# RubenMovsesyan/DiPs

Hardware: AMD Instinct MI355X
Metric: frames/s + achieved HBM GB/s (% of roofline), 4K RGB8, 1/2/4/8 GPUs (higher is better)
Workload: dtype u8

## Files before the change

### dips_amd/csrc/dips_abi.hip

```cpp
#include <hip/hip_runtime.h>

#include <cmath>
#include <cstring>
#include <mutex>
#include <new>
#include <string>

#include "dips_handle.h"

namespace {

std::mutex g_err_mu;
std::string g_create_err;

void set_create_err(const std::string& m) {
    std::lock_guard<std::mutex> lk(g_err_mu);
    g_create_err = m;
}

dips_status validate_params(const dips_params* p, std::string* why) {
    if (p->spatial_window_size < 1 || p->spatial_window_size > 11) {
        *why = "spatial_window_size must be in [1, 11] (dips_shader.wgsl:27 MAX_WIN_SIZE_SQUARE = 11*11)";
        return DIPS_ERR_INVALID;
    }
    if (p->chroma_filter > 3u) {
        *why = "chroma_filter must be 0..3 (dips/src/lib.rs:43-61)";
        return DIPS_ERR_INVALID;
    }
    if (p->mode > 1u) {
        *why = "mode must be DIPS_MODE_OVERALL or DIPS_MODE_PER_FRAME";
        return DIPS_ERR_INVALID;
    }
    if (p->format != DIPS_FMT_GRAY8 && p->format != DIPS_FMT_RGB8 && p->format != DIPS_FMT_RGBA8) {
        *why = "format must be DIPS_FMT_GRAY8, DIPS_FMT_RGB8 or DIPS_FMT_RGBA8";
        return DIPS_ERR_INVALID;
    }
    if (!(p->tau >= 0.0f) || std::isinf(p->tau)) {
        *why = "tau must be finite and >= 0";
        return DIPS_ERR_INVALID;
    }
    if (!std::isfinite(p->sensitivity)) {
        *why = "sensitivity must be finite";
        return DIPS_ERR_INVALID;
    }
    return DIPS_OK;
}

}

namespace dips_abi {

void note_error(dips_handle* h, const char* msg) noexcept {
    if (!h) return;
    try {
        h->err = msg;
    } catch (...) {
    }
}

void note_error(CreateTag, const char* msg) noexcept {
    try {
        set_create_err(msg);
    } catch (...) {
    }
}

}

namespace dips_internal {

dips_status fail(dips_handle* h, dips_status st, const std::string& msg) {
    if (h) h->err = msg;
    return st;
}

dips_status hip_fail(dips_handle* h, hipError_t e, const char* what) {
    std::string m = std::string(what) + ": " + hipGetErrorString(e);
    return fail(h, e == hipErrorOutOfMemory ? DIPS_ERR_NOMEM : DIPS_ERR_HIP, m);
}

dips_status bind(dips_handle* h) {
    if (!h) return DIPS_ERR_INVALID;
    hipError_t e = hipSetDevice(h->device);
    if (e != hipSuccess) return hip_fail(h, e, "hipSetDevice");
    return DIPS_OK;
}

hipEvent_t take_event(dips_handle* h) {
    if (!h->ev_free.empty()) {
        hipEvent_t e = h->ev_free.back();
        h->ev_free.pop_back();
        return e;
    }
    hipEvent_t e = nullptr;
    if (hipEventCreate(&e) != hipSuccess) return nullptr;
    return e;
}

int occupancy_blocks(dips_handle* h, const void* kernel) {
    auto it = h->occupancy.find(kernel);
    if (it != h->occupancy.end()) return it->second;
    int nb = 0;
    if (hipOccupancyMaxActiveBlocksPerMultiprocessor(&nb, kernel, 256, 0) != hipSuccess || nb < 1) nb = 1;
    h->occupancy[kernel] = nb;
    return nb;
}

}

using dips_abi::guard;
using namespace dips_internal;

namespace dips_abi {
int current_device() noexcept {
    int d = -1;
    return hipGetDevice(&d) == hipSuccess ? d : -1;
}
void set_device(int dev) noexcept { (void)hipSetDevice(dev); }
}

extern "C" {

int dips_abi_version(void) {
    return guard(nullptr, [&]() -> int { return DIPS_ABI_VERSION; });
}

dips_status dips_params_default(dips_params* p) {
    return guard(nullptr, [&]() -> dips_status {
        if (!p) return DIPS_ERR_INVALID;
        std::memset(p, 0, sizeof(*p));
        p->colorize = 0;
        p->spatial_window_size = 1;
        p->sensitivity = 5.0f;
        p->filter_type = DIPS_FILTER_UNFILTERED;
        p->chroma_filter = DIPS_CHROMA_NONE;
        p->mode = DIPS_MODE_OVERALL;
        p->format = DIPS_FMT_RGB8;
        p->tau = 0.0f;
        p->flags = 0;
        return DIPS_OK;
    });
}

dips_status dips_create(const dips_params* params, int device, dips_handle** out) {
    return guard(dips_abi::CreateTag{}, [&]() -> dips_status {
        if (!out) return DIPS_ERR_INVALID;
        *out = nullptr;
        dips_params p;
        if (params) p = *params;
        else dips_params_default(&p);
        std::string why;
        if (validate_params(&p, &why) != DIPS_OK) {
            set_create_err(why);
            return DIPS_ERR_INVALID;
        }
        int count = 0;
        hipError_t e = hipGetDeviceCount(&count);
        if (e != hipSuccess || count <= 0 || device < 0 || device >= count) {
            set_create_err(std::string("no HIP device ") + std::to_string(device) + " (" +
                           (e == hipSuccess ? std::to_string(count) + " visible" : hipGetErrorString(e)) + ")");
            return DIPS_ERR_NODEVICE;
        }
        dips_handle* h = new (std::nothrow) dips_handle();
        if (!h) return DIPS_ERR_NOMEM;
        h->p = p;
        h->device = device;
        e = hipSetDevice(device);
        if (e == hipSuccess) e = hipDeviceGetAttribute(&h->cu_count, hipDeviceAttributeMultiprocessorCount, device);
        if (e == hipSuccess) e = hipStreamCreateWithFlags(&h->own_stream, hipStreamDefault);
        if (e == hipSuccess) e = hipStreamCreateWithFlags(&h->copy_stream, hipStreamNonBlocking);
        for (int i = 0; i < 3 && e == hipSuccess; ++i) {
            e = hipEventCreateWithFlags(&h->copy_done[i], hipEventDisableTiming);
            if (e == hipSuccess) e = hipEventCreateWithFlags(&h->kernel_done[i], hipEventDisableTiming);
        }
        if (e != hipSuccess) {
            set_create_err(std::string("HIP initialisation failed: ") + hipGetErrorString(e));
            dips_destroy(h);
            return DIPS_ERR_HIP;
        }
        h->stream = h->own_stream;
        *out = h;
        return DIPS_OK;
    });
}

void dips_destroy(dips_handle* h) {
    guard(h, [&]() -> void {
        if (!h) return;
        (void)hipSetDevice(h->device);
        if (h->stream) (void)hipStreamSynchronize(h->stream);
        if (h->copy_stream) (void)hipStreamSynchronize(h->copy_stream);
        if (h->comm_stream) (void)hipStreamSynchronize(h->comm_stream);
        for (auto& pr : h->ev_pending) {
            (void)hipEventDestroy(pr.first);
            (void)hipEventDestroy(pr.second);
        }
        for (auto e : h->ev_free) (void)hipEventDestroy(e);
        for (int i = 0; i < 3; ++i) {
            if (h->copy_done[i]) (void)hipEventDestroy(h->copy_done[i]);
            if (h->kernel_done[i]) (void)hipEventDestroy(h->kernel_done[i]);
            h->ring[i].release();
        }
        h->ring_ref.release();
        h->pinned[0].release();
        h->pinned[1].release();
        h->partials.release();
        h->stage_frames.release();
        h->stage_ref.release();
        h->stage_series.release();
        h->stage_map.release();
        for (auto& s : h->slots) s.release();
        for (auto& s : h->slots_alt) s.release();
        h->pipe.release();
        h->pieces.release();
        h->up_pieces.release();
        h->probe_out.release();
        h->times_parts.release();
        h->cc_scratch.release();
        h->io_out.release();
        h->raw.release();
        h->filtered.release();
        h->cb_lut.release();
        h->gray_lut.release();
        h->start.release();
        h->out.release();
        h->io.release();
        h->shard_ref.release();
        h->shard_halo.release();
        h->shard_send.release();
        h->shard_recv.release();
        h->shard_send_frame.release();
        if (h->comm_stream) (void)hipStreamDestroy(h->comm_stream);
        if (h->shard_ev_in) (void)hipEventDestroy(h->shard_ev_in);
        if (h->shard_ev_halo) (void)hipEventDestroy(h->shard_ev_halo);
        if (h->switch_ev) (void)hipEventDestroy(h->switch_ev);
        if (h->join_ev) (void)hipEventDestroy(h->join_ev);
        if (h->own_stream) (void)hipStreamDestroy(h->own_stream);
        if (h->copy_stream) (void)hipStreamDestroy(h->copy_stream);
        delete h;
    });
}

const char* dips_last_error(const dips_handle* h) {
    return guard(h, [&]() -> const char* {
        if (h) return h->err.c_str();
        thread_local std::string copy;
        std::lock_guard<std::mutex> lk(g_err_mu);
        copy = g_create_err;
        return copy.c_str();
    });
}

dips_status dips_set_stream(dips_handle* h, void* stream) {
    return guard(h, [&]() -> dips_status {
        if (!h) return DIPS_ERR_INVALID;
        hipStream_t next = stream ? static_cast<hipStream_t>(stream) : h->own_stream;
        if (next == h->stream) return DIPS_OK;
        dips_status st = bind(h);
        if (st != DIPS_OK) return st;
        st = flush_pending(h);
        if (st != DIPS_OK) return st;
        if (!h->switch_ev) DIPS_HIP(h, hipEventCreateWithFlags(&h->switch_ev, hipEventDisableTiming));
        DIPS_HIP(h, hipEventRecord(h->switch_ev, h->stream));
        DIPS_HIP(h, hipStreamWaitEvent(next, h->switch_ev, 0));
        h->stream = next;
        return DIPS_OK;
    });
}

dips_status dips_synchronize(dips_handle* h) {
    return guard(h, [&]() -> dips_status {
        dips_status st = bind(h);
        if (st != DIPS_OK) return st;
        st = flush_pending(h);
        if (st != DIPS_OK) return st;
        DIPS_HIP(h, hipStreamSynchronize(h->stream));
        return DIPS_OK;
    });
}

dips_status dips_kernel_time(dips_handle* h, double* total_ms, uint64_t* launches) {
    return guard(h, [&]() -> dips_status {
        dips_status st = bind(h);
        if (st != DIPS_OK) return st;
        for (auto& pr : h->ev_pending) {
            DIPS_HIP(h, hipEventSynchronize(pr.second));
            float ms = 0.0f;
            DIPS_HIP(h, hipEventElapsedTime(&ms, pr.first, pr.second));
            h->t_ms += ms;
            h->t_launches += 1;
            if (h->t_each.size() >= dips_handle::kTimeKeep)
                h->t_each.erase(h->t_each.begin(), h->t_each.begin() + dips_handle::kTimeKeep / 2);
            h->t_each.push_back(ms);
            h->ev_free.push_back(pr.first);
            h->ev_free.push_back(pr.second);
        }
        h->ev_pending.clear();
        if (total_ms) *total_ms = h->t_ms;
        if (launches) *launches = h->t_launches;
        return DIPS_OK;
    });
}

dips_status dips_kernel_time_reset(dips_handle* h) {
    return guard(h, [&]() -> dips_status {
        dips_status st = dips_kernel_time(h, nullptr, nullptr);
        if (st != DIPS_OK) return st;
        h->t_ms = 0.0;
        h->t_launches = 0;
        h->t_each.clear();
        return DIPS_OK;
    });
}

dips_status dips_kernel_time_each(dips_handle* h, double* ms_each, uint64_t cap, uint64_t* launches) {
    return guard(h, [&]() -> dips_status {
        dips_status st = dips_kernel_time(h, nullptr, nullptr);
        if (st != DIPS_OK) return st;
        const uint64_t n = h->t_each.size();
// ... 13 lines not shown
```

### dips_amd/csrc/dips_handle.h

```cpp
#pragma once

#include <hip/hip_runtime.h>

#include <cstdint>
#include <map>
#include <string>
#include <utility>
#include <vector>

#include "../../include/dips_hip.h"
#include "abi_guard.h"
#include "host_buffers.h"
#include "host_stream.h"

struct dips_handle {
    dips_params p{};
    int device = 0;
    int cu_count = 0;
    hipStream_t own_stream = nullptr;
    hipStream_t stream = nullptr;
    hipStream_t copy_stream = nullptr;
    hipEvent_t switch_ev = nullptr;
    hipEvent_t join_ev = nullptr;
    std::string err;

    dips_host::DevBuf partials, stage_frames, stage_ref, stage_series, stage_map;
    dips_host::DevBuf probe_out;
    dips_host::DevBuf times_parts;
    dips_host::DevBuf cc_scratch;
    std::map<const void*, int> occupancy;

    dips_host::DevBuf ring[3];
    dips_host::DevBuf ring_ref;
    dips_host::HostPinned pinned[2];
    hipEvent_t copy_done[3] = {nullptr, nullptr, nullptr};
    hipEvent_t kernel_done[3] = {nullptr, nullptr, nullptr};

    static constexpr size_t kTimeKeep = 65536;
    std::vector<std::pair<hipEvent_t, hipEvent_t>> ev_pending;
    std::vector<hipEvent_t> ev_free;
    double t_ms = 0.0;
    uint64_t t_launches = 0;
    std::vector<double> t_each;

    uint32_t width = 0, height = 0;
    int n_queued = 0;
    bool main_init = false;
    uint32_t ring_idx = 0;
    uint32_t uniform_idx = 0;
    dips_host::DevBuf slots[4], raw, start, out;
    dips_host::HostPinned io;
    uint64_t added = 0;
    dips_host::DevBuf slots_alt[4];
    dips_host::DevBuf filtered;
    dips_host::StreamPipe pipe;
    dips_host::PieceEvents pieces;
    dips_host::PieceEvents up_pieces;
    dips_host::HostPinned io_out;
    dips_host::CallPhases cb_phases;
    bool cb_phases_valid = false;
    bool pending = false;
    uint32_t pending_slot = 0;
    dips_host::DirectGeom pend_geom;
    int pend_key = 0;
    bool slot_raw[4] = {false, false, false, false};
    int cb_occupancy = 0;
    dips_host::DevBuf gray_lut;
    bool gray_lut_valid = false;
    float gray_lut_tau = 0.0f;
    dips_host::DevBuf cb_lut;
    bool cb_lut_valid = false;
    uint32_t cb_lut_filter = 0, cb_lut_col = 0;
    float cb_lut_k = 0.0f;

    dips_host::DevBuf shard_ref, shard_halo, shard_send, shard_recv;
    dips_host::DevBuf shard_send_frame;
    hipStream_t comm_stream = nullptr;
    hipEvent_t shard_ev_in = nullptr, shard_ev_halo = nullptr;
    const uint8_t* shard_last_ref = nullptr;
    uint64_t shard_last_bytes = 0;

    bool crosscheck() const { return (p.flags & DIPS_FLAG_CROSSCHECK) != 0; }
};

namespace dips_internal {

dips_status fail(dips_handle* h, dips_status st, const std::string& msg);
dips_status hip_fail(dips_handle* h, hipError_t e, const char* what);
dips_status bind(dips_handle* h);
hipEvent_t take_event(dips_handle* h);
int occupancy_blocks(dips_handle* h, const void* kernel);
dips_status flush_pending(dips_handle* h);
dips_status run_series_device(dips_handle* h, uint32_t width, uint32_t height, const uint8_t* frames,
                              uint32_t n_frames, const uint8_t* ref0, dips_series_entry* series, uint8_t* map,
                              hipStream_t s);
dips_status compat_resume_impl(dips_handle* h, uint32_t width, uint32_t height, const uint8_t* start_rgba,
                               const uint8_t* halo, uint64_t t0, bool dev);
dips_status run_series_streamed(dips_handle* h, uint32_t width, uint32_t height, const uint8_t* host_frames,
                                uint32_t n_frames, const uint8_t* ref_dev, dips_series_entry* series_dev,
                                uint32_t chunk_frames);
uint64_t series_waves(dips_handle* h, uint32_t width, uint32_t height, uint32_t n_frames, bool env_cap);

}

#define DIPS_HIP(h, call)                                                     \
    do {                                                                      \
        hipError_t e_ = (call);                                               \
        if (e_ != hipSuccess) return dips_internal::hip_fail((h), e_, #call); \
    } while (0)

namespace dips_internal {

struct KernelSpan {
    dips_handle* h;
    hipEvent_t e0 = nullptr, e1 = nullptr;
    explicit KernelSpan(dips_handle* handle) : h(handle) {}
    KernelSpan(const KernelSpan&) = delete;
    KernelSpan& operator=(const KernelSpan&) = delete;
    ~KernelSpan() {
        try {
            if (e0) h->ev_free.push_back(e0);
            if (e1) h->ev_free.push_back(e1);
        } catch (...) {
        }
    }
    dips_status take() {
        if (!(h->p.flags & DIPS_FLAG_TIME_KERNEL) || e0) return DIPS_OK;
        e0 = take_event(h);
        e1 = take_event(h);
        if (!e0 || !e1) return fail(h, DIPS_ERR_HIP, "hipEventCreate failed");
        return DIPS_OK;
    }
    dips_status begin(hipStream_t s) {
        const dips_status st = take();
        if (st != DIPS_OK || !e0) return st;
        DIPS_HIP(h, hipEventRecord(e0, s));
        return DIPS_OK;
    }
    dips_status end(hipStream_t s) {
        if (!e0) return DIPS_OK;
        DIPS_HIP(h, hipEventRecord(e1, s));
        h->ev_pending.emplace_back(e0, e1);
        e0 = e1 = nullptr;
        return DIPS_OK;
    }
};

}

#define DIPS_TRY(expr)                      \
    do {                                    \
        const dips_status st_ = (expr);     \
        if (st_ != DIPS_OK) return st_;     \
    } while (0)
```

### dips_amd/csrc/dips_kernels.h

```cpp
#pragma once

#include <hip/hip_runtime.h>
#include <stdint.h>

#include "../../include/dips_hip.h"

namespace dips {

constexpr bool fits_grid256(uint64_t n) { return n <= (1ull << 32) - 256u; }

constexpr int kUnrollRGB = 4;
constexpr int kUnrollGray = 2;
constexpr int kUnrollV2 = 4;
constexpr int kUnrollV2Rgb = 5;
template <int C>
constexpr int v2_unroll() { return C == 3 ? kUnrollV2Rgb : kUnrollV2; }
#ifndef DIPS_UNROLL_GRAY_LUT
#define DIPS_UNROLL_GRAY_LUT 4
#endif
constexpr int kUnrollGrayLut = DIPS_UNROLL_GRAY_LUT;
constexpr uint32_t kGrayLutWaves = 16;
constexpr size_t kGrayLutBytes = 131072;
constexpr size_t kGrayLutAllocBytes = kGrayLutBytes + 256;
#ifndef DIPS_DEPTH_RGB
#define DIPS_DEPTH_RGB 2
#endif
#ifndef DIPS_DEPTH_GRAY
#define DIPS_DEPTH_GRAY 2
#endif
constexpr int kDepthRGB = DIPS_DEPTH_RGB;
constexpr int kDepthGray = DIPS_DEPTH_GRAY;

struct SeriesArgs {
    const uint8_t* frames;
    const uint8_t* ref0;
    uint8_t* dmap;
    uint64_t* partials;
    uint64_t items;
    uint32_t frame_bytes;
    uint32_t vec_bytes;
    uint32_t n_frames;
    uint32_t n_tiles;
    uint32_t n_waves;
    float thr;
    const void* lut;
    uint32_t part_frames;
    uint32_t probe_min;
    uint32_t probe_hi;
    uint32_t probe_spread;
    uint64_t* zero;
    uint32_t zero_n;
};

struct GenericArgs {
    const uint8_t* frames;
    const uint8_t* ref0;
    uint8_t* dmap;
    dips_series_entry* series;
    uint64_t frame_bytes;
    uint64_t n_px;
    uint64_t px0;
    uint32_t n_frames;
    uint32_t blocks_per_frame;
    uint32_t mode;
    uint32_t chroma;
    float tau;
};

struct GridSpec {
    uint32_t x, y, w, h;
    uint32_t rows, cols;
};

struct GridRect {
    uint32_t x, y, w, h;
};

__host__ __device__ inline uint32_t grid_edge(uint32_t x0, uint32_t extent, uint32_t n, uint32_t i) {
    return x0 + (uint32_t)((uint64_t)i * extent / n);
}

__host__ __device__ inline GridRect grid_cell_rect(const GridSpec& g, uint32_t row, uint32_t col) {
    GridRect r;
    r.x = grid_edge(g.x, g.w, g.cols, col);
    r.y = grid_edge(g.y, g.h, g.rows, row);
    r.w = grid_edge(g.x, g.w, g.cols, col + 1) - r.x;
    r.h = grid_edge(g.y, g.h, g.rows, row + 1) - r.y;
    return r;
}

struct GridArgs {
    const uint8_t* frames;
    const uint8_t* ref0;
    uint64_t* partials;
    uint64_t* zero;
    uint32_t zero_n;
    uint32_t frame_bytes;
    uint32_t width;
    uint32_t n_frames;
    uint32_t tiles_per_cell;
    uint32_t n_tiles;
    uint32_t n_waves;
    uint32_t part_frames;
    float thr;
    GridSpec g;
};

struct GridGenericArgs {
    const uint8_t* frames;
    const uint8_t* ref0;
    dips_series_entry* cells;
    uint64_t frame_bytes;
    uint32_t width;
    uint32_t n_frames;
    uint32_t segs_per_cell;
    uint32_t out_stride;
    uint32_t out_base;
    uint32_t mode;
    uint32_t chroma;
    float tau;
    GridSpec g;
};

#ifndef DIPS_UNROLL_PIX
#define DIPS_UNROLL_PIX 2
#endif
constexpr int kUnrollPix = DIPS_UNROLL_PIX;
constexpr uint32_t kPixMaxPart = 2048;
struct PixArgs {
    const uint8_t* frames;
    const uint8_t* ref0;
    dips_series_entry* sums;
    uint32_t frame_bytes;
    uint32_t width;
    uint32_t n_frames;
    uint32_t n_tiles;
    uint32_t n_waves;
    uint32_t part_frames;
    uint32_t out_mode;
    float thr;
    GridRect roi;
};

struct PixGenericArgs {
    const uint8_t* frames;
    const uint8_t* ref0;
    dips_series_entry* sums;
    uint64_t frame_bytes;
    uint32_t width;
    uint32_t n_frames;
    uint32_t mode;
    uint32_t chroma;
    float tau;
    uint32_t accumulate;
    uint32_t roi_x, roi_y, roi_w;
    GridRect rect;
};

#ifndef DIPS_UNROLL_MASK
#define DIPS_UNROLL_MASK 4
#endif
constexpr int kUnrollMask = DIPS_UNROLL_MASK;
struct MaskArgs {
    const uint8_t* frames;
    const uint8_t* ref0;
    uint8_t* mask;
    uint32_t frame_bytes;
    uint32_t mask_frame_bytes;
    uint32_t width;
    uint32_t n_frames;
    uint32_t n_tiles;
    uint32_t n_waves;
    uint32_t part_frames;
    float thr;
    GridRect roi;
};

struct MaskGenericArgs {
    const uint8_t* frames;
    const uint8_t* ref0;
    uint8_t* mask;
    uint64_t frame_bytes;
    uint64_t mask_frame_bytes;
    uint32_t width;
    uint32_t t0, n_frames;
    uint32_t mode;
    uint32_t chroma;
    float tau;
    uint32_t row0, n_rows, word0, n_words;
    GridRect roi;
};

#ifndef DIPS_UNROLL_TIMES
#define DIPS_UNROLL_TIMES 2
#endif
constexpr int kUnrollTimes = DIPS_UNROLL_TIMES;
struct TimesArgs {
// ... 389 lines not shown
```

### dips_amd/csrc/series_abi.hip

```cpp
#include <hip/hip_runtime.h>

#include <algorithm>
#include <cmath>
#include <cstdlib>
#include <cstring>

#include "series_host.h"

using dips_abi::guard;
using namespace dips_internal;

namespace {

using dips_sched::FastGeom;

FastGeom fast_geometry(dips_handle* h, uint32_t width, uint32_t height, uint32_t n_frames, int C, bool pf,
                       bool map, bool align = false, int isi = 0, bool env_cap = true) {
    const void* k = dips::series_fast_kernel_ptr(C, C == 1 ? 0 : (int)h->p.chroma_filter, pf, map, align, isi);
    return dips_sched::fast_geometry(width, height, n_frames, C, dips::pixels_per_vec(C), dips::fast_unroll(C),
                                     resident_waves(h, k, env_cap));
}

constexpr double kGrayAutoMin = 0.25, kGrayAutoHi = 0.9;
constexpr uint32_t kGrayAutoSpread = 48;
constexpr int kGrayLayout = 4;

bool gray_lut_enabled(const dips_handle* h) { return !h->crosscheck(); }

FastGeom gray_lut_geometry(dips_handle* h, uint32_t width, uint32_t height, uint32_t n_frames, bool env_cap = true) {
    return dips_sched::gray_lut_geometry(width, height, n_frames, dips::kUnrollGrayLut, dips::kGrayLutWaves,
                                         h->p.mode == DIPS_MODE_PER_FRAME,
                                         resident_at(h, dips::kGrayLutWaves / 4u, env_cap));
}

dips_status ensure_gray_lut(dips_handle* h, hipStream_t s) {
    if (h->gray_lut_valid && h->gray_lut_tau == h->p.tau) return DIPS_OK;
    DIPS_HIP(h, h->gray_lut.ensure(2 * dips::kGrayLutAllocBytes));
    DIPS_HIP(h, dips::launch_gray_lut(h->gray_lut.as<uint8_t>(), h->p.tau, kGrayLayout, s));
    h->gray_lut_valid = true;
    h->gray_lut_tau = h->p.tau;
    return DIPS_OK;
}

}

namespace dips_internal {

dips_status run_series_device(dips_handle* h, uint32_t width, uint32_t height, const uint8_t* frames,
                              uint32_t n_frames, const uint8_t* ref0, dips_series_entry* series, uint8_t* map,
                              hipStream_t s) {
    const int C = (int)h->p.format;
    const bool pf = h->p.mode == DIPS_MODE_PER_FRAME;
    const uint64_t npx = (uint64_t)width * height;
    const uint64_t fb = npx * (uint64_t)C;
    FastGeom g;
    const bool glut = C == 1 && gray_lut_enabled(h);
    const bool align = (C == 3 || C == 4) && ((((uintptr_t)frames | (uintptr_t)fb | (uintptr_t)ref0) & 3u) != 0u);
    const int isi = series_isi_form(h);
    if (!(h->p.flags & DIPS_FLAG_FORCE_GENERIC))
        g = glut ? gray_lut_geometry(h, width, height, n_frames)
                 : fast_geometry(h, width, height, n_frames, C, pf, map != nullptr, align, isi);
    const bool kzero = g.ok && (glut || C != 1) && n_frames < (1u << 30);
    if (!kzero) DIPS_HIP(h, hipMemsetAsync(series, 0, sizeof(dips_series_entry) * (size_t)n_frames, s));
    auto launch_generic = [&](uint64_t px0) -> dips_status {
        const uint64_t bpf = (npx - px0 + 255u) / 256u;
        if (bpf >= (1ull << 32))
            return fail(h, DIPS_ERR_INVALID, "frame too large for the generic kernel (2^40 pixels)");
        dips::GenericArgs a{};
        a.frames = frames;
        a.ref0 = ref0;
        a.dmap = map;
        a.series = series;
        a.frame_bytes = fb;
        a.n_px = npx;
        a.px0 = px0;
        a.n_frames = n_frames;
        a.blocks_per_frame = (uint32_t)bpf;
        a.mode = h->p.mode;
        a.chroma = C == 1 ? 0u : h->p.chroma_filter;
        a.tau = h->p.tau;
        DIPS_HIP(h, dips::launch_series_generic(a, C, s));
        return DIPS_OK;
    };

    KernelSpan span(h);
    DIPS_TRY(span.take());
    if (g.ok && glut) DIPS_TRY(ensure_gray_lut(h, s));
    DIPS_TRY(span.begin(s));
    if (g.ok) {
        DIPS_HIP(h, h->partials.ensure((size_t)g.items * 16u));
        dips::SeriesArgs a{};
        if (glut) {
            a.probe_min = std::max(1u, (uint32_t)std::ceil(kGrayAutoMin * 1024.0));
            if (h->p.flags & DIPS_FLAG_GRAY_BAND_TABLE) a.probe_min = 0u;
            else if (h->p.flags & DIPS_FLAG_GRAY_PAIR_TABLE) a.probe_min = 1025u;
            a.probe_hi = (uint32_t)std::ceil(kGrayAutoHi * 1024.0);
            a.probe_spread = kGrayAutoSpread;
        }
        if (kzero) {
            a.zero = reinterpret_cast<uint64_t*>(series);
            a.zero_n = 4u * n_frames;
        }
        a.frames = frames;
        a.ref0 = ref0;
        a.dmap = map;
        a.partials = h->partials.as<uint64_t>();
        a.items = g.items;
        a.frame_bytes = (uint32_t)fb;
        a.vec_bytes = (uint32_t)g.vec_bytes;
        a.n_frames = n_frames;
        a.n_tiles = (uint32_t)g.n_tiles;
        a.n_waves = (uint32_t)g.n_waves;
        a.thr = dips::series_threshold(C, h->p.tau, isi);
        a.part_frames = g.part_frames;
        if (glut) {
            a.lut = h->gray_lut.p;
            DIPS_HIP(h, dips::launch_series_gray_lut(a, pf, map != nullptr, (uint32_t)g.blocks, s));
        } else {
            DIPS_HIP(h, dips::launch_series_fast(a, C, C == 1 ? 0 : (int)h->p.chroma_filter, pf, map != nullptr,
                                                 (uint32_t)g.blocks, s, align, isi));
        }
        if (g.tail_px0 < npx) DIPS_TRY(launch_generic(g.tail_px0));
    } else {
        DIPS_TRY(launch_generic(0));
    }
    DIPS_TRY(span.end(s));
    if (g.ok)
        DIPS_HIP(h, dips::launch_series_reduce(h->partials.as<uint64_t>(), n_frames, (uint32_t)g.n_tiles,
                                               C == 1 ? (glut ? 2 : 1) : 0, series, s));
    return DIPS_OK;
}

uint64_t series_waves(dips_handle* h, uint32_t width, uint32_t height, uint32_t n_frames, bool env_cap) {
    const int C = (int)h->p.format;
    FastGeom g = C == 1 && gray_lut_enabled(h)
                     ? gray_lut_geometry(h, width, height, n_frames, env_cap)
                     : fast_geometry(h, width, height, n_frames, C, h->p.mode == DIPS_MODE_PER_FRAME, false, false,
                                     series_isi_form(h), env_cap);
    return g.ok ? g.n_waves : 0;
}

dips_status run_series_streamed(dips_handle* h, uint32_t width, uint32_t height, const uint8_t* host_frames,
                                uint32_t n_frames, const uint8_t* ref_dev, dips_series_entry* series_dev,
                                uint32_t chunk_frames) {
    if (n_frames == 0) return DIPS_OK;
    const bool pf = h->p.mode == DIPS_MODE_PER_FRAME;
    const size_t fb = (size_t)width * height * (size_t)h->p.format;
    uint32_t chunk = chunk_frames;
    if (chunk == 0) {
        const size_t target = 256u << 20;
        chunk = (uint32_t)(target / fb);
        if (chunk < 1) chunk = 1;
    }
    if (chunk > n_frames) chunk = n_frames;
    const size_t cbytes = fb * chunk;
    for (auto& r : h->ring) DIPS_HIP(h, r.ensure(cbytes));
    DIPS_HIP(h, h->ring_ref.ensure(fb));
    for (auto& pn : h->pinned) DIPS_HIP(h, pn.ensure(cbytes));
    DIPS_HIP(h, hipStreamSynchronize(h->copy_stream));
    DIPS_HIP(h, hipStreamSynchronize(h->stream));
    const uint32_t n_chunks = (n_frames + chunk - 1) / chunk;
    for (uint32_t k = 0; k < n_chunks; ++k) {
        const uint32_t b = k % 3u, hb = k % 2u;
        const uint32_t f0 = k * chunk;
        const uint32_t nk = (f0 + chunk <= n_frames) ? chunk : n_frames - f0;
        if (k >= 2) DIPS_HIP(h, hipEventSynchronize(h->copy_done[(k - 2) % 3u]));
        dips_host::staged_copy(static_cast<uint8_t*>(h->pinned[hb].p), host_frames + (size_t)f0 * fb,
                               (size_t)nk * fb);
        if (k >= 2) DIPS_HIP(h, hipStreamWaitEvent(h->copy_stream, h->kernel_done[(k - 2) % 3u], 0));
        DIPS_HIP(h, dips_host::pipe_h2d(h->ring[b].p, h->pinned[hb].p, (size_t)nk * fb, h->copy_stream, true));
        DIPS_HIP(h, hipEventRecord(h->copy_done[b], h->copy_stream));
        DIPS_HIP(h, hipStreamWaitEvent(h->stream, h->copy_done[b], 0));
        const uint8_t* frames_dev = h->ring[b].as<uint8_t>();
        const uint8_t* ref;
        if (pf) {
            if (k == 0) ref = ref_dev ? ref_dev : frames_dev;
            else ref = h->ring[(k - 1) % 3u].as<uint8_t>() + (size_t)(chunk - 1) * fb;
        } else {
            if (k == 0 && !ref_dev)
                DIPS_HIP(h, hipMemcpyAsync(h->ring_ref.p, frames_dev, fb, hipMemcpyDeviceToDevice, h->stream));
            ref = ref_dev ? ref_dev : h->ring_ref.as<uint8_t>();
        }
        dips_status st = run_series_device(h, width, height, frames_dev, nk, ref, series_dev + f0, nullptr, h->stream);
        if (st != DIPS_OK) return st;
        DIPS_HIP(h, hipEventRecord(h->kernel_done[b], h->stream));
    }
    return DIPS_OK;
}

}

namespace {

template <typename Launch>
dips_status time_leg(dips_handle* h, double* ms, Launch&& launch) {
    DIPS_HIP(h, h->probe_out.ensure(256));
    hipEvent_t e0 = take_event(h), e1 = take_event(h);
    if (!e0 || !e1) return fail(h, DIPS_ERR_HIP, "hipEventCreate failed");
    DIPS_HIP(h, hipEventRecord(e0, h->stream));
    DIPS_HIP(h, launch());
    DIPS_HIP(h, hipEventRecord(e1, h->stream));
    DIPS_HIP(h, hipEventSynchronize(e1));
    float t = 0.0f;
    DIPS_HIP(h, hipEventElapsedTime(&t, e0, e1));
    *ms = t;
    h->ev_free.push_back(e0);
    h->ev_free.push_back(e1);
    return DIPS_OK;
}

}

extern "C" {

dips_status dips_diff_series(dips_handle* h, uint32_t width, uint32_t height, const uint8_t* frames,
                             uint32_t n_frames, const uint8_t* ref, dips_series_entry* series, uint8_t* map) {
    return guard(h, [&]() -> dips_status {
        dips_status st = bind(h);
        if (st != DIPS_OK) return st;
        if (n_frames == 0) return DIPS_OK;
        if (!frames || !series || width == 0 || height == 0)
            return fail(h, DIPS_ERR_INVALID, "diff_series: null or empty argument");
        const uint64_t fb = frame_bytes(h, width, height);
        if (h->p.flags & DIPS_FLAG_DEVICE_PTRS)
            return run_series_device(h, width, height, frames, n_frames, ref ? ref : frames, series, map, h->stream);
        const size_t total = (size_t)fb * n_frames;
        const uint8_t *frames_dev, *ref_dev;
        DIPS_TRY(stage_host_frames(h, frames, total, ref, fb, h->stage_series,
                                   sizeof(dips_series_entry) * (size_t)n_frames, &frames_dev, &ref_dev));
        uint8_t* map_dev = nullptr;
        if (map) {
            DIPS_HIP(h, h->stage_map.ensure(total));
            map_dev = h->stage_map.as<uint8_t>();
        }
        st = run_series_device(h, width, height, frames_dev, n_frames, ref_dev,
                               h->stage_series.as<dips_series_entry>(), map_dev, h->stream);
        if (st != DIPS_OK) return st;
        DIPS_HIP(h, hipMemcpyAsync(series, h->stage_series.p, sizeof(dips_series_entry) * (size_t)n_frames,
                                   hipMemcpyDeviceToHost, h->stream));
        if (map) DIPS_HIP(h, hipMemcpyAsync(map, map_dev, total, hipMemcpyDeviceToHost, h->stream));
        DIPS_HIP(h, hipStreamSynchronize(h->stream));
        return DIPS_OK;
    });
}

dips_status dips_diff_series_streamed(dips_handle* h, uint32_t width, uint32_t height, const uint8_t* host_frames,
                                      uint32_t n_frames, const uint8_t* host_ref, dips_series_entry* series,
                                      uint32_t chunk_frames) {
    return guard(h, [&]() -> dips_status {
        dips_status st = bind(h);
        if (st != DIPS_OK) return st;
        if (n_frames == 0) return DIPS_OK;
        if (!host_frames || !series || width == 0 || height == 0)
            return fail(h, DIPS_ERR_INVALID, "diff_series_streamed: null or empty argument");
        const size_t fb = (size_t)width * height * (size_t)h->p.format;
        DIPS_HIP(h, h->stage_series.ensure(sizeof(dips_series_entry) * (size_t)n_frames));
        dips_series_entry* series_dev = h->stage_series.as<dips_series_entry>();
        const uint8_t* ref_dev = nullptr;
        if (host_ref) {
            DIPS_HIP(h, hipStreamSynchronize(h->stream));
            DIPS_HIP(h, h->ring_ref.ensure(fb));
            DIPS_HIP(h, h->pinned[1].ensure(fb));
            DIPS_HIP(h, hipStreamSynchronize(h->copy_stream));
            std::memcpy(h->pinned[1].p, host_ref, fb);
            DIPS_HIP(h, hipMemcpyAsync(h->ring_ref.p, h->pinned[1].p, fb, hipMemcpyHostToDevice, h->copy_stream));
            DIPS_HIP(h, hipStreamSynchronize(h->copy_stream));
            ref_dev = h->ring_ref.as<uint8_t>();
        }
        st = run_series_streamed(h, width, height, host_frames, n_frames, ref_dev, series_dev, chunk_frames);
        if (st != DIPS_OK) return st;
        DIPS_HIP(h, hipMemcpyAsync(series, series_dev, sizeof(dips_series_entry) * (size_t)n_frames,
                                   hipMemcpyDeviceToHost, h->stream));
        DIPS_HIP(h, hipStreamSynchronize(h->stream));
        return DIPS_OK;
    });
}

dips_status dips_synth_frames(dips_handle* h, uint32_t width, uint32_t height, uint64_t seed, uint64_t t0,
                              uint32_t n_frames, uint8_t* dst) {
    return guard(h, [&]() -> dips_status {
        dips_status st = bind(h);
        if (st != DIPS_OK) return st;
        if (n_frames == 0) return DIPS_OK;
        if (!dst || width == 0 || height == 0)
            return fail(h, DIPS_ERR_INVALID, "synth_frames: null or empty argument");
        dips::SynthArgs a{};
        a.dst = dst;
        a.channels = h->p.format;
        a.width = width;
        a.height = height;
        a.frame_bytes = (uint64_t)width * height * a.channels;
        a.total_bytes = a.frame_bytes * n_frames;
        a.seed = seed;
        a.t0 = t0;
        a.radius = height / 8u > 0 ? height / 8u : 1u;
        DIPS_HIP(h, dips::launch_synth(a, h->stream));
        return DIPS_OK;
    });
}

dips_status dips_read_ceiling(dips_handle* h, const uint8_t* dev_bytes, uint64_t bytes, double* ms) {
    return guard(h, [&]() -> dips_status {
        dips_status st = bind(h);
        if (st != DIPS_OK) return st;
        if (!dev_bytes || !ms) return fail(h, DIPS_ERR_INVALID, "read_ceiling: null argument");
        return time_leg(h, ms, [&]() {
            return dips::launch_read_ceiling(dev_bytes, bytes, h->probe_out.as<uint32_t>(), h->stream);
        });
    });
}

dips_status dips_read_ceiling_walk(dips_handle* h, const uint8_t* dev_frames, uint32_t width, uint32_t height,
                                   uint32_t n_frames, double* ms) {
    return guard(h, [&]() -> dips_status {
        dips_status st = bind(h);
        if (st != DIPS_OK) return st;
        if (!dev_frames || !ms) return fail(h, DIPS_ERR_INVALID, "read_ceiling_walk: null argument");
        const int C = (int)h->p.format;
        if (C != 3 && C != 4) return fail(h, DIPS_ERR_INVALID, "read_ceiling_walk: RGB8 / RGBA8 only");
        FastGeom g = fast_geometry(h, width, height, n_frames, C, h->p.mode == DIPS_MODE_PER_FRAME, false, false,
                                   series_isi_form(h));
        if (!g.ok) return fail(h, DIPS_ERR_INVALID, "read_ceiling_walk: shape not eligible for the series kernel");
        dips::SeriesArgs a{};
        a.frames = dev_frames;
        a.items = g.items;
        a.frame_bytes = (uint32_t)((uint64_t)width * height * (uint64_t)C);
        a.vec_bytes = (uint32_t)g.vec_bytes;
        a.n_frames = n_frames;
        a.n_tiles = (uint32_t)g.n_tiles;
        a.n_waves = (uint32_t)g.n_waves;
        a.part_frames = g.part_frames;
        return time_leg(h, ms, [&]() {
            return dips::launch_read_walk(a, C == 3 ? 12 : 16, (uint32_t)g.blocks, h->probe_out.as<uint32_t>(),
                                          h->stream);
        });
    });
}

dips_status dips_series_geometry(dips_handle* h, uint32_t width, uint32_t height, uint32_t n_frames,
                                 uint64_t* waves, uint64_t* tiles, uint64_t* partial_bytes) {
    return guard(h, [&]() -> dips_status {
        dips_status st = bind(h);
        if (st != DIPS_OK) return st;
        const int C = (int)h->p.format;
        FastGeom g = C == 1 && gray_lut_enabled(h)
                         ? gray_lut_geometry(h, width, height, n_frames)
                         : fast_geometry(h, width, height, n_frames, C, h->p.mode == DIPS_MODE_PER_FRAME, false,
                                         false, series_isi_form(h));
        if (waves) *waves = g.ok ? g.n_waves : 0;
        if (tiles) *tiles = g.ok ? g.n_tiles : 0;
        if (partial_bytes) *partial_bytes = g.ok ? g.n_tiles * 16u : 0;
        return g.ok ? DIPS_OK : fail(h, DIPS_ERR_INVALID, "shape not eligible for the fast kernel");
    });
}

}
```

### dips_amd/csrc/series_host.h

```cpp
#pragma once

#include <cstdlib>

#include "dips_handle.h"
#include "dips_kernels.h"
#include "series_sched.h"

namespace dips_internal {

using dips_sched::mask_words_per_row;

inline uint64_t waves_per_simd(uint64_t occupancy, bool env_cap) {
    if (env_cap) {
        if (const char* cap = std::getenv("DIPS_SERIES_WAVES_PER_SIMD")) {
            const unsigned long c = std::strtoul(cap, nullptr, 10);
            if (c >= 1 && c < occupancy) return c;
        }
    }
    return occupancy;
}

inline uint64_t resident_at(const dips_handle* h, uint64_t occupancy, bool env_cap = true) {
    return waves_per_simd(occupancy, env_cap) * (uint64_t)h->cu_count * 4u;
}

inline uint64_t resident_waves(dips_handle* h, const void* kernel, bool env_cap = true) {
    return kernel ? resident_at(h, (uint64_t)occupancy_blocks(h, kernel), env_cap) : 0u;
}

inline uint64_t pixel_part_pin() {
    const char* pin = std::getenv("DIPS_PIXEL_PART_FRAMES");
    return pin ? std::strtoul(pin, nullptr, 10) : 0u;
}

inline int series_isi_form(const dips_handle* h) {
    const int C = (int)h->p.format;
    if (C == 1 || h->crosscheck() || !dips::series_v2_isi(h->p.tau)) return 0;
    return 1;
}

inline bool regional_fast_path(const dips_handle* h) {
    return h->p.format != DIPS_FMT_GRAY8 && !(h->p.flags & DIPS_FLAG_FORCE_GENERIC) && !h->crosscheck();
}

inline uint64_t frame_bytes(const dips_handle* h, uint32_t width, uint32_t height) {
    return (uint64_t)width * height * (uint64_t)h->p.format;
}

template <typename Row>
dips_status for_frame_end_tail_rows(uint32_t width, uint32_t height, const dips::GridSpec& g, Row&& row) {
    return dips_sched::for_frame_end_tail_rows(width, height, g.x, g.y, g.w, g.h, row);
}

inline dips_status stage_host_frames(dips_handle* h, const uint8_t* frames, size_t total, const uint8_t* ref, size_t fb,
                                     dips_host::DevBuf& out, size_t out_bytes, const uint8_t** frames_dev,
                                     const uint8_t** ref_dev) {
    DIPS_HIP(h, h->stage_frames.ensure(total));
    DIPS_HIP(h, out.ensure(out_bytes));
    if (total) DIPS_HIP(h, hipMemcpyAsync(h->stage_frames.p, frames, total, hipMemcpyHostToDevice, h->stream));
    *frames_dev = total ? h->stage_frames.as<uint8_t>() : nullptr;
    *ref_dev = h->stage_frames.as<uint8_t>();
    if (ref) {
        DIPS_HIP(h, h->stage_ref.ensure(fb));
        DIPS_HIP(h, hipMemcpyAsync(h->stage_ref.p, ref, fb, hipMemcpyHostToDevice, h->stream));
        *ref_dev = h->stage_ref.as<uint8_t>();
    }
    return DIPS_OK;
}

}
```

### dips_amd/csrc/series_v2.hip

```cpp
#include "series_v2_frame.h"

namespace dips {

template <int C, int U, bool PF, bool MAP, bool ALIGN = false>
constexpr int v2_min_waves() {
    return ALIGN ? (MAP ? 1 : (U >= 5 ? 3 : 4)) : ((C == 3 && PF && !MAP) ? (U <= 2 ? 8 : (U == 3 ? 6 : (U == 4 ? 5 : 4))) : 1);
}

template <int N, int L>
__device__ __forceinline__ void funnel(uint32_t (&v)[L], uint32_t sh) {
    static_assert(L > N, "a funnel needs the dword after the vec");
#pragma unroll
    for (int k = 0; k < N; ++k) v[k] = __builtin_amdgcn_alignbyte(v[k + 1], v[k], sh);
}

template <int C, int CH, int U, bool PF, bool MAP, int AUX, int SAUX, int SCHED = 0, bool ALIGN = false,
          int ISI = 0, int WPB = 4>
__device__ __forceinline__ void series_v2_body(const SeriesArgs& a) {
    using F = Fmt<C>;
    static_assert(!ALIGN || C == 3 || C == 4, "the aligned-load form is the RGB8 / RGBA8 one");
    constexpr bool A4 = ALIGN && C == 4;
    constexpr int LW = (ALIGN && C == 3) ? F::NDW + 1 : F::NDW;
    static_assert(U * 64 * F::VB <= 4096, "vec offsets must fit the 12-bit immediate");
    zero_series(a);
    const uint32_t lane = threadIdx.x & 63u;
    const uint32_t wave = __builtin_amdgcn_readfirstlane(blockIdx.x * (uint32_t)WPB + (threadIdx.x >> 6));
    if (wave >= a.n_waves) return;
    const uint32_t fb = a.frame_bytes, vb = a.vec_bytes;
    const uint32_t rec_off8 = (lane & 7u) == 0u ? (lane >> 5) * 16u + ((lane >> 3) & 3u) * 4u : 0x80000000u;
    const uint32_t rec_off4 = (lane & 15u) == 0u ? (lane >> 4) * 4u : 0x80000000u;

    uint64_t i = (uint64_t)wave * a.items / a.n_waves;
    const uint64_t iend = (uint64_t)(wave + 1) * a.items / a.n_waves;
    const bool parts = SCHED == 1 || a.part_frames != 0u;
    const uint32_t plen = parts ? a.part_frames : 1u;
    const uint64_t pitems = parts ? (uint64_t)((a.n_frames + plen - 1) / plen) * a.n_tiles : 0u;
    uint64_t it = wave;
    while (true) {
        uint32_t tile, t0, tend;
        if (!parts) {
            if (i >= iend) break;
            tile = (uint32_t)(i / a.n_frames);
            t0 = (uint32_t)(i - (uint64_t)tile * a.n_frames);
            const uint64_t remaining = iend - i;
            tend = (uint32_t)((uint64_t)a.n_frames < t0 + remaining ? (uint64_t)a.n_frames : t0 + remaining);
            i += tend - t0;
        } else {
            if (it >= pitems) break;
            const uint32_t part = (uint32_t)(it / a.n_tiles);
            tile = (uint32_t)(it - (uint64_t)part * a.n_tiles);
            t0 = part * plen;
            tend = min(a.n_frames, t0 + plen);
            it += a.n_waves;
        }
        const uint32_t n = tend - t0;
        const uint32_t tlast = tend - 1;
        const uint32_t voff = (tile * U * 64u + lane) * (uint32_t)F::VB;
        const __amdgpu_buffer_rsrc_t rpart =
            make_rsrc(a.partials + 2 * (uint64_t)tile * a.n_frames, a.n_frames * 16u);

        const uint32_t tile_end = (tile + 1u) * U * 64u * (uint32_t)F::VB;
        auto load_at = [&](const uint8_t* p, uint32_t (&dst)[U][LW], uint32_t* sh, uint32_t* tl) {
            if constexpr (ALIGN) {
                const uint32_t d = (uint32_t)(uintptr_t)p & 3u;
                *sh = d;
                const __amdgpu_buffer_rsrc_t r = make_rsrc(p - d, (vb + d + 3u) & ~3u);
#pragma unroll
                for (int u = 0; u < U; ++u) {
                    const u32x4 x = __builtin_amdgcn_raw_buffer_load_b128(r, voff + (uint32_t)(u * 64 * F::VB), 0, AUX);
                    dst[u][0] = x.x;
                    dst[u][1] = x.y;
                    dst[u][2] = x.z;
                    dst[u][3] = x.w;
                }
                if constexpr (A4) *tl = __builtin_amdgcn_raw_buffer_load_b32(r, tile_end, 0, AUX);
            } else {
                const __amdgpu_buffer_rsrc_t r = make_rsrc(p, vb);
#pragma unroll
                for (int u = 0; u < U; ++u) load_vec<C, AUX>(r, voff + (uint32_t)(u * 64 * F::VB), dst[u]);
            }
        };
        uint32_t sh[4] = {0u, 0u, 0u, 0u};
        uint32_t tl[4] = {0u, 0u, 0u, 0u};
        auto load_frame = [&](uint32_t tf, uint32_t (&dst)[U][LW], uint32_t* shp, uint32_t* tlp) {
#ifdef DIPS_PROBE_SAMEFRAME
            tf = t0;
#endif
            load_at(a.frames + (uint64_t)min(tf, tlast) * fb, dst, shp, tlp);
        };

        uint32_t buf[4][U][LW];
        uint32_t rb[U][LW];
        St2 st[U];
        uint32_t keep[U];
#pragma unroll
        for (int u = 0; u < U; ++u) keep[u] = voff + (uint32_t)(u * 64 * F::VB) < vb ? 0xFFFFFFFFu : 0u;
        const bool lane63 = lane == 63u;
        auto realign = [&](uint32_t (&v)[U][LW], uint32_t shv, uint32_t tlv) {
            if constexpr (ALIGN) {
#pragma unroll
                for (int u = 0; u < U; ++u) {
                    if constexpr (A4) {
                        uint32_t nx = DIPS_DPP(v[u][0], 0x130);
                        const uint32_t l63 = u + 1 < U ? (uint32_t)__builtin_amdgcn_readlane((int)v[u + 1][0], 0)
                                                       : __builtin_amdgcn_readfirstlane(tlv);
                        nx = lane63 ? l63 : nx;
#pragma unroll
                        for (int k = 0; k < 3; ++k) v[u][k] = __builtin_amdgcn_alignbyte(v[u][k + 1], v[u][k], shv);
                        v[u][3] = __builtin_amdgcn_alignbyte(nx, v[u][3], shv);
                    } else {
                        funnel<F::NDW>(v[u], shv);
                    }
                    v[u][0] &= keep[u];
                }
            }
        };
        auto settle = [&](int j) {
            if constexpr (ALIGN) realign(buf[j], sh[j], tl[j]);
        };
        {
            const uint8_t* rp = PF ? (t0 == 0 ? a.ref0 : a.frames + (uint64_t)(t0 - 1) * fb) : a.ref0;
            uint32_t (&dref)[U][LW] = PF ? buf[0] : rb;
            uint32_t rsh = 0, rtl = 0;
            load_at(rp, dref, &rsh, &rtl);
            if constexpr (PF) {
                load_frame(t0, buf[1], &sh[1], &tl[1]);
                load_frame(t0 + 1, buf[2], &sh[2], &tl[2]);
                load_frame(t0 + 2, buf[3], &sh[3], &tl[3]);
            } else {
                load_frame(t0, buf[0], &sh[0], &tl[0]);
                load_frame(t0 + 1, buf[1], &sh[1], &tl[1]);
                load_frame(t0 + 2, buf[2], &sh[2], &tl[2]);
                load_frame(t0 + 3, buf[3], &sh[3], &tl[3]);
            }
            if constexpr (ALIGN) realign(dref, rsh, rtl);
#pragma unroll
            for (int u = 0; u < U; ++u) {
                uint32_t dv[F::NDW];
#pragma unroll
                for (int k2 = 0; k2 < F::NDW; ++k2) dv[k2] = dref[u][k2];
                derive_v2<C, CH, (ISI != 0)>(dv, st[u]);
            }
        }

        uint32_t k = 0;
        for (; k + 4 <= n; k += 4) {
#pragma unroll
            for (int h = 0; h < 2; ++h) {
                uint32_t v[8], c0, c1;
#pragma unroll
                for (int q = 0; q < 2; ++q) {
                    const int j = 2 * h + q;
                    const uint32_t tf = t0 + k + (uint32_t)j;
                    if constexpr (PF) {
                        settle((j + 1) & 3);
                        frame_v2<C, CH, U, PF, MAP, SAUX, LW, LW, ISI>(a, st, buf[j], buf[(j + 1) & 3], voff, tf,
                                                                  v + 4 * q, q ? c1 : c0);
                        __builtin_amdgcn_sched_barrier(0);
                        load_frame(tf + 3, buf[j], &sh[j], &tl[j]);
                    } else {
                        settle(j);
                        frame_v2<C, CH, U, PF, MAP, SAUX, LW, LW, ISI>(a, st, rb, buf[j], voff, tf, v + 4 * q,
                                                                  q ? c1 : c0);
                        __builtin_amdgcn_sched_barrier(0);
                        load_frame(tf + 4, buf[j], &sh[j], &tl[j]);
                    }
                }
                const uint32_t y = wave_sum8_lanes(v, lane);
                store_pair(rpart, t0 + k + 2 * h, rec_off8, lane, y, c0, c1);
            }
        }
#pragma unroll
        for (int j = 0; j < 3; ++j) {
            if (k + (uint32_t)j < n) {
                uint32_t v[4], c;
                const uint32_t tf = t0 + k + (uint32_t)j;
                if constexpr (PF) {
                    settle(j + 1);
                    frame_v2<C, CH, U, PF, MAP, SAUX, LW, LW, ISI>(a, st, buf[j], buf[j + 1], voff, tf, v, c);
                } else {
                    settle(j);
                    frame_v2<C, CH, U, PF, MAP, SAUX, LW, LW, ISI>(a, st, rb, buf[j], voff, tf, v, c);
                }
                const uint32_t y = wave_sum4_lanes(v);
                store_one(rpart, tf, rec_off4, lane, y, c);
            }
        }
    }
}

template <int C, int CH, int U, bool PF, bool MAP, bool ALIGN = false, int ISI = 0>
__global__ __launch_bounds__(256, (v2_min_waves<C, U, PF, MAP, ALIGN>())) void series_v2_kernel(SeriesArgs a) {
    series_v2_body<C, CH, U, PF, MAP, kAuxNT, kAuxNT, 0, ALIGN, ISI>(a);
}

template <int C, int CH, bool PF, bool MAP, bool ALIGN, int ISI>
static const void* v2_ptr() {
    return reinterpret_cast<const void*>(&series_v2_kernel<C, CH, v2_unroll<C>(), PF, MAP, ALIGN && (C == 3 || C == 4), ISI>);
}

template <int C, bool ALIGN, int ISI>
static const void* pick_v2(int chroma, bool pf, bool map) {
#define DIPS_PICK_V2(CHV)                                                                                   \
    case CHV:                                                                                               \
        return pf ? (map ? v2_ptr<C, CHV, true, true, ALIGN, ISI>() : v2_ptr<C, CHV, true, false, ALIGN, ISI>()) \
                  : (map ? v2_ptr<C, CHV, false, true, ALIGN, ISI>()                                        \
                         : v2_ptr<C, CHV, false, false, ALIGN, ISI>());
    switch (chroma) {
        DIPS_PICK_V2(0)
        DIPS_PICK_V2(1)
        DIPS_PICK_V2(2)
        DIPS_PICK_V2(3)
        default: return nullptr;
    }
#undef DIPS_PICK_V2
}

const void* series_v2_kernel_ptr(int channels, int chroma, bool per_frame, bool map, bool align, int isi) {
    switch (channels) {
        case 3:
            if (isi == 1)
                return align ? pick_v2<3, true, 1>(chroma, per_frame, map) : pick_v2<3, false, 1>(chroma, per_frame, map);
            return align ? pick_v2<3, true, 0>(chroma, per_frame, map) : pick_v2<3, false, 0>(chroma, per_frame, map);
        case 4:
            if (isi == 1)
                return align ? pick_v2<4, true, 1>(chroma, per_frame, map) : pick_v2<4, false, 1>(chroma, per_frame, map);
            return align ? pick_v2<4, true, 0>(chroma, per_frame, map) : pick_v2<4, false, 0>(chroma, per_frame, map);
        default: return nullptr;
    }
}

bool series_v2_isi(float tau) { return tau >= kIsiMinTau; }

}
```

Measured before the change: 240,400.

## Add integer pre-screen to skip float intensity path in per-frame RGB series kernel

Adds a screened variant of the per-frame RGB8 series kernel. It keeps a packed 16-bit max+min lightness state per pixel and uses a cheap integer threshold test with a wave ballot to decide whether the full floating-point derive and threshold work is needed for each unrolled vector. Waves with no candidate pixels skip the expensive path. It also sets a fixed launch bound, adds a host screen level and an env toggle, and adds a new form code 3. The risk is divergence and extra integer work when many pixels pass the screen, plus correctness depending on the screen bound being conservative.

```diff
diff --git a/dips_amd/csrc/dips_abi.hip b/dips_amd/csrc/dips_abi.hip
--- a/dips_amd/csrc/dips_abi.hip
+++ b/dips_amd/csrc/dips_abi.hip
@@ -1,6 +1,7 @@
 #include <hip/hip_runtime.h>
 
 #include <cmath>
+#include <cstdlib>
 #include <cstring>
 #include <mutex>
 #include <new>
@@ -165,6 +166,7 @@
         if (!h) return DIPS_ERR_NOMEM;
         h->p = p;
         h->device = device;
+        if (const char* scr = std::getenv("DIPS_SERIES_SCREEN")) h->series_screen = std::strtol(scr, nullptr, 10) != 0;
         e = hipSetDevice(device);
         if (e == hipSuccess) e = hipDeviceGetAttribute(&h->cu_count, hipDeviceAttributeMultiprocessorCount, device);
         if (e == hipSuccess) e = hipStreamCreateWithFlags(&h->own_stream, hipStreamDefault);
diff --git a/dips_amd/csrc/dips_handle.h b/dips_amd/csrc/dips_handle.h
--- a/dips_amd/csrc/dips_handle.h
+++ b/dips_amd/csrc/dips_handle.h
@@ -80,6 +80,8 @@
     const uint8_t* shard_last_ref = nullptr;
     uint64_t shard_last_bytes = 0;
 
+    bool series_screen = true;
+
     bool crosscheck() const { return (p.flags & DIPS_FLAG_CROSSCHECK) != 0; }
 };
 
diff --git a/dips_amd/csrc/dips_kernels.h b/dips_amd/csrc/dips_kernels.h
--- a/dips_amd/csrc/dips_kernels.h
+++ b/dips_amd/csrc/dips_kernels.h
@@ -43,6 +43,7 @@
     uint32_t n_tiles;
     uint32_t n_waves;
     float thr;
+    uint32_t screen;
     const void* lut;
     uint32_t part_frames;
     uint32_t probe_min;
diff --git a/dips_amd/csrc/series_abi.hip b/dips_amd/csrc/series_abi.hip
--- a/dips_amd/csrc/series_abi.hip
+++ b/dips_amd/csrc/series_abi.hip
@@ -56,7 +56,7 @@
     FastGeom g;
     const bool glut = C == 1 && gray_lut_enabled(h);
     const bool align = (C == 3 || C == 4) && ((((uintptr_t)frames | (uintptr_t)fb | (uintptr_t)ref0) & 3u) != 0u);
-    const int isi = series_isi_form(h);
+    const int isi = series_v2_form(h);
     if (!(h->p.flags & DIPS_FLAG_FORCE_GENERIC))
         g = glut ? gray_lut_geometry(h, width, height, n_frames)
                  : fast_geometry(h, width, height, n_frames, C, pf, map != nullptr, align, isi);
@@ -112,6 +112,7 @@
         a.n_tiles = (uint32_t)g.n_tiles;
         a.n_waves = (uint32_t)g.n_waves;
         a.thr = dips::series_threshold(C, h->p.tau, isi);
+        a.screen = (uint32_t)std::max(0, dips::series_screen_level(h->p.tau));
         a.part_frames = g.part_frames;
         if (glut) {
             a.lut = h->gray_lut.p;
@@ -136,7 +137,7 @@
     FastGeom g = C == 1 && gray_lut_enabled(h)
                      ? gray_lut_geometry(h, width, height, n_frames, env_cap)
                      : fast_geometry(h, width, height, n_frames, C, h->p.mode == DIPS_MODE_PER_FRAME, false, false,
-                                     series_isi_form(h), env_cap);
+                                     series_v2_form(h), env_cap);
     return g.ok ? g.n_waves : 0;
 }
 
@@ -319,7 +320,7 @@
         const int C = (int)h->p.format;
         if (C != 3 && C != 4) return fail(h, DIPS_ERR_INVALID, "read_ceiling_walk: RGB8 / RGBA8 only");
         FastGeom g = fast_geometry(h, width, height, n_frames, C, h->p.mode == DIPS_MODE_PER_FRAME, false, false,
-                                   series_isi_form(h));
+                                   series_v2_form(h));
         if (!g.ok) return fail(h, DIPS_ERR_INVALID, "read_ceiling_walk: shape not eligible for the series kernel");
         dips::SeriesArgs a{};
         a.frames = dev_frames;
@@ -346,7 +347,7 @@
         FastGeom g = C == 1 && gray_lut_enabled(h)
                          ? gray_lut_geometry(h, width, height, n_frames)
                          : fast_geometry(h, width, height, n_frames, C, h->p.mode == DIPS_MODE_PER_FRAME, false,
-                                         false, series_isi_form(h));
+                                         false, series_v2_form(h));
         if (waves) *waves = g.ok ? g.n_waves : 0;
         if (tiles) *tiles = g.ok ? g.n_tiles : 0;
         if (partial_bytes) *partial_bytes = g.ok ? g.n_tiles * 16u : 0;
diff --git a/dips_amd/csrc/series_host.h b/dips_amd/csrc/series_host.h
--- a/dips_amd/csrc/series_host.h
+++ b/dips_amd/csrc/series_host.h
@@ -5,6 +5,7 @@
 #include "dips_handle.h"
 #include "dips_kernels.h"
 #include "series_sched.h"
+#include "series_screen_rule.h"
 
 namespace dips_internal {
 
@@ -39,6 +40,11 @@
     return 1;
 }
 
+inline int series_v2_form(const dips_handle* h) {
+    const int isi = series_isi_form(h);
+    return isi == 1 && !h->series_screen ? 3 : isi;
+}
+
 inline bool regional_fast_path(const dips_handle* h) {
     return h->p.format != DIPS_FMT_GRAY8 && !(h->p.flags & DIPS_FLAG_FORCE_GENERIC) && !h->crosscheck();
 }
diff --git a/dips_amd/csrc/series_screen_rule.h b/dips_amd/csrc/series_screen_rule.h
--- /dev/null
+++ b/dips_amd/csrc/series_screen_rule.h
@@ -0,0 +1,15 @@
+#pragma once
+
+#include <cmath>
+
+namespace dips {
+
+inline int series_screen_level(float tau) {
+    const double lim = 510.0 * (double)tau - 3e-4;
+    if (!(lim > 0.0)) return -1;
+    if (lim > 510.0) return 510;
+    const double c = std::ceil(lim);
+    return (int)c - 1;
+}
+
+}
diff --git a/dips_amd/csrc/series_v2.hip b/dips_amd/csrc/series_v2.hip
--- a/dips_amd/csrc/series_v2.hip
+++ b/dips_amd/csrc/series_v2.hip
@@ -1,10 +1,15 @@
-#include "series_v2_frame.h"
+#include "series_v2_screen.h"
 
 namespace dips {
 
 template <int C, int U, bool PF, bool MAP, bool ALIGN = false>
 constexpr int v2_min_waves() {
     return ALIGN ? (MAP ? 1 : (U >= 5 ? 3 : 4)) : ((C == 3 && PF && !MAP) ? (U <= 2 ? 8 : (U == 3 ? 6 : (U == 4 ? 5 : 4))) : 1);
+}
+
+template <int C, int CH, bool PF, bool MAP, bool ALIGN, int ISI>
+constexpr bool v2_screened() {
+    return ISI == 1 && C == 3 && CH == 0 && PF && !MAP && !ALIGN;
 }
 
 template <int N, int L>
@@ -21,6 +26,8 @@
     static_assert(!ALIGN || C == 3 || C == 4, "the aligned-load form is the RGB8 / RGBA8 one");
     constexpr bool A4 = ALIGN && C == 4;
     constexpr int LW = (ALIGN && C == 3) ? F::NDW + 1 : F::NDW;
+    constexpr bool SCR = v2_screened<C, CH, PF, MAP, ALIGN, ISI>();
+    constexpr int FISI = ISI != 0 ? 1 : 0;
     static_assert(U * 64 * F::VB <= 4096, "vec offsets must fit the 12-bit immediate");
     zero_series(a);
     const uint32_t lane = threadIdx.x & 63u;
@@ -91,7 +98,17 @@
 
         uint32_t buf[4][U][LW];
         uint32_t rb[U][LW];
-        St2 st[U];
+        St2 st[SCR ? 1 : U];
+        uint32_t jst[SCR ? U : 1][2];
+        ScreenLevel lv{};
+        if constexpr (SCR) lv = screen_level(a);
+        auto frame = [&](const uint32_t (&rv)[U][LW], const uint32_t (&cv)[U][LW], uint32_t tf, uint32_t* vals,
+                         uint32_t& cnt) __attribute__((always_inline)) {
+            if constexpr (SCR)
+                frame_v2_screen<U, PF>(a, lv, jst, rv, cv, vals, cnt);
+            else
+                frame_v2<C, CH, U, PF, MAP, SAUX, LW, LW, FISI>(a, st, rv, cv, voff, tf, vals, cnt);
+        };
         uint32_t keep[U];
 #pragma unroll
         for (int u = 0; u < U; ++u) keep[u] = voff + (uint32_t)(u * 64 * F::VB) < vb ? 0xFFFFFFFFu : 0u;
@@ -139,7 +156,10 @@
                 uint32_t dv[F::NDW];
 #pragma unroll
                 for (int k2 = 0; k2 < F::NDW; ++k2) dv[k2] = dref[u][k2];
-                derive_v2<C, CH, (ISI != 0)>(dv, st[u]);
+                if constexpr (SCR)
+                    derive_j(dv, jst[u]);
+                else
+                    derive_v2<C, CH, (ISI != 0)>(dv, st[u]);
             }
         }
 
@@ -154,14 +174,12 @@
                     const uint32_t tf = t0 + k + (uint32_t)j;
                     if constexpr (PF) {
                         settle((j + 1) & 3);
-                        frame_v2<C, CH, U, PF, MAP, SAUX, LW, LW, ISI>(a, st, buf[j], buf[(j + 1) & 3], voff, tf,
-                                                                  v + 4 * q, q ? c1 : c0);
+                        frame(buf[j], buf[(j + 1) & 3], tf, v + 4 * q, q ? c1 : c0);
                         __builtin_amdgcn_sched_barrier(0);
                         load_frame(tf + 3, buf[j], &sh[j], &tl[j]);
                     } else {
                         settle(j);
-                        frame_v2<C, CH, U, PF, MAP, SAUX, LW, LW, ISI>(a, st, rb, buf[j], voff, tf, v + 4 * q,
-                                                                  q ? c1 : c0);
+                        frame(rb, buf[j], tf, v + 4 * q, q ? c1 : c0);
                         __builtin_amdgcn_sched_barrier(0);
                         load_frame(tf + 4, buf[j], &sh[j], &tl[j]);
                     }
@@ -177,10 +195,10 @@
                 const uint32_t tf = t0 + k + (uint32_t)j;
                 if constexpr (PF) {
                     settle(j + 1);
-                    frame_v2<C, CH, U, PF, MAP, SAUX, LW, LW, ISI>(a, st, buf[j], buf[j + 1], voff, tf, v, c);
+                    frame(buf[j], buf[j + 1], tf, v, c);
                 } else {
                     settle(j);
-                    frame_v2<C, CH, U, PF, MAP, SAUX, LW, LW, ISI>(a, st, rb, buf[j], voff, tf, v, c);
+                    frame(rb, buf[j], tf, v, c);
                 }
                 const uint32_t y = wave_sum4_lanes(v);
                 store_one(rpart, tf, rec_off4, lane, y, c);
@@ -190,7 +208,8 @@
 }
 
 template <int C, int CH, int U, bool PF, bool MAP, bool ALIGN = false, int ISI = 0>
-__global__ __launch_bounds__(256, (v2_min_waves<C, U, PF, MAP, ALIGN>())) void series_v2_kernel(SeriesArgs a) {
+__global__ __launch_bounds__(256, (v2_screened<C, CH, PF, MAP, ALIGN, ISI>() ? 4 : v2_min_waves<C, U, PF, MAP, ALIGN>()))
+void series_v2_kernel(SeriesArgs a) {
     series_v2_body<C, CH, U, PF, MAP, kAuxNT, kAuxNT, 0, ALIGN, ISI>(a);
 }
 
@@ -217,6 +236,10 @@
 }
 
 const void* series_v2_kernel_ptr(int channels, int chroma, bool per_frame, bool map, bool align, int isi) {
+    if (isi == 3) {
+        if (channels == 3 && chroma == 0 && per_frame && !map && !align) return v2_ptr<3, 0, true, false, false, 3>();
+        isi = 1;
+    }
     switch (channels) {
         case 3:
             if (isi == 1)
diff --git a/dips_amd/csrc/series_v2_screen.h b/dips_amd/csrc/series_v2_screen.h
--- /dev/null
+++ b/dips_amd/csrc/series_v2_screen.h
@@ -0,0 +1,90 @@
+#pragma once
+
+#include "series_v2_frame.h"
+
+namespace dips {
+
+__device__ __forceinline__ void derive_j(const uint32_t (&d)[3], uint32_t (&j)[2]) {
+    u16x2 r[2], g[2], b[2];
+    pair_planes<3>(d, r, g, b);
+#pragma unroll
+    for (int k = 0; k < 2; ++k) {
+        const h2 rh = __builtin_bit_cast(h2, r[k]), gh = __builtin_bit_cast(h2, g[k]), bh = __builtin_bit_cast(h2, b[k]);
+        const h2 mx = __builtin_elementwise_maximum(__builtin_elementwise_maximum(rh, gh), bh);
+        const h2 mn = __builtin_elementwise_minimum(__builtin_elementwise_minimum(rh, gh), bh);
+        j[k] = as_u32(__builtin_bit_cast(u16x2, mx) + __builtin_bit_cast(u16x2, mn));
+    }
+}
+
+struct ScreenLevel {
+    uint32_t s, s2;
+};
+__device__ __forceinline__ ScreenLevel screen_level(const SeriesArgs& a) {
+    const uint32_t s = __builtin_amdgcn_readfirstlane(a.screen);
+    return {s * 0x00010001u, s * 0x00020002u};
+}
+
+template <int U, bool PF>
+__device__ __forceinline__ void frame_v2_screen(const SeriesArgs& a, ScreenLevel lv, uint32_t (&jst)[U][2],
+                                                const uint32_t (&rb)[U][3], const uint32_t (&cur)[U][3],
+                                                uint32_t* vals, uint32_t& cnt) {
+    uint32_t sad = 0, sj = 0, c = 0;
+    uint32_t si0 = 0, si1 = 0;
+    uint64_t hit[U];
+#pragma unroll
+    for (int u = 0; u < U; ++u) {
+#pragma unroll
+        for (int k = 0; k < 3; ++k) sad = __builtin_amdgcn_sad_u8(cur[u][k], rb[u][k], sad);
+        uint32_t jc[2];
+        derive_j(cur[u], jc);
+        u16x2 far = {0, 0};
+#pragma unroll
+        for (int k = 0; k < 2; ++k) {
+            asm volatile("v_sad_u16 %0, %1, %2, %0" : "+v"(sj) : "v"(jc[k]), "v"(jst[u][k]));
+            const u16x2 d = as_u16x2(jc[k]) - as_u16x2(jst[u][k]) + as_u16x2(lv.s);
+            far = k == 0 ? d : __builtin_elementwise_max(far, d);
+        }
+        const uint32_t over = as_u32(__builtin_elementwise_sub_sat(far, as_u16x2(lv.s2)));
+        hit[u] = __ballot(over != 0u);
+        if constexpr (PF) {
+            jst[u][0] = jc[0];
+            jst[u][1] = jc[1];
+        }
+    }
+#pragma unroll
+    for (int u = 0; u < U; ++u) {
+        if (hit[u] != 0ull) {
+            uint32_t rv[3], cv[3];
+#pragma unroll
+            for (int k = 0; k < 3; ++k) {
+                rv[k] = rb[u][k];
+                cv[k] = cur[u][k];
+                asm volatile("" : "+v"(rv[k]), "+v"(cv[k]));
+            }
+            St2 r, n;
+            derive_v2<3, 0, true>(rv, r);
+            derive_v2<3, 0, true>(cv, n);
+#pragma unroll
+            for (int k = 0; k < 2; ++k) {
+                const f32x2 d = n.i[k] - r.i[k];
+                const float a0 = fabsf(d.x), a1 = fabsf(d.y);
+                const bool s0 = a0 > a.thr, s1 = a1 > a.thr;
+                const uint64_t m0 = __ballot(s0), m1 = __ballot(s1);
+                c += (uint32_t)__builtin_popcountll(m0) + (uint32_t)__builtin_popcountll(m1);
+                const uint32_t v = (uint32_t)(s0 ? a0 : 0.0f) + (uint32_t)(s1 ? a1 : 0.0f);
+                if (u < U / 2)
+                    si0 += v;
+                else
+                    si1 += v;
+            }
+        }
+    }
+    vals[0] = sad;
+    vals[1] = sj;
+    const uint64_t s64 = (uint64_t)si0 + (uint64_t)si1;
+    vals[2] = (uint32_t)(s64 >> 11);
+    vals[3] = ((uint32_t)s64 & 0x7FFu) << 4;
+    cnt = c;
+}
+
+}
```

Measured after the change: 244,700, median of 6. 1.8% higher.
